# BioJulia/Kmers.jl

Measured on NVIDIA B200. Metric: canonical 31-mers+hash/sec, higher is better.
Workload: dtype u64

## Files before the change

### kmers.jl_b200/csrc/api.cu

```cuda
#include <algorithm>
#include <cstdio>
#include <cstring>
#include <new>
#include <vector>

#include "fourbit.h"
#include "plan.h"

namespace kmc {

int32_t fail_cuda(kmc_ctx *ctx, cudaError_t e, const char *what)
{
    if (ctx) {
        char buf[512];
        snprintf(buf, sizeof buf, "%s: %s (%s)", what, cudaGetErrorName(e), cudaGetErrorString(e));
        ctx->last_error = buf;
    }
    return -static_cast<int32_t>(e);
}

int32_t fail(kmc_ctx *ctx, int32_t code, const char *msg)
{
    if (ctx) ctx->last_error = msg;
    return code;
}

ExtractLaunchFn get_launcher(const Geometry &ge, int mode, bool hash, bool ragged)
{
    switch (ge.n_limbs) {
    case 1: return get_extract_launcher_n1(ge.nx, mode, hash, ragged);
    case 2: return get_extract_launcher_n2(ge.nx, mode, hash, ragged);
    case 3: return get_extract_launcher_n3(ge.nx, mode, hash, ragged);
    case 4: return get_extract_launcher_n4(ge.nx, mode, hash, ragged);
    }
    return nullptr;
}

ExtractLaunchFn get_digest_launcher(const Geometry &ge, int mode, bool hash, bool ragged)
{
    switch (ge.n_limbs) {
    case 1: return get_digest_launcher_n1(ge.nx, mode, hash, ragged);
    case 2: return get_digest_launcher_n2(ge.nx, mode, hash, ragged);
    }
    return nullptr;
}

namespace {

bool aligned32(const void *p) { return (reinterpret_cast<uintptr_t>(p) & 31) == 0; }

__global__ void fill_uniform_offsets_kernel(uint64_t *out, uint64_t n_plus_1, uint64_t step)
{
    uint64_t i = static_cast<uint64_t>(blockIdx.x) * blockDim.x + threadIdx.x;
    if (i < n_plus_1) out[i] = i * step;
}

}

cudaError_t fill_uniform_offsets(uint64_t *out, uint64_t n_plus_1, uint64_t step, cudaStream_t stream)
{
    fill_uniform_offsets_kernel<<<static_cast<unsigned>((n_plus_1 + 255) / 256), 256, 0, stream>>>(out, n_plus_1, step);
    return cudaGetLastError();
}

int32_t check_common(kmc_ctx *ctx, const kmc_seqs *s, int32_t k)
{
    if (!ctx) return KMC_E_BAD_ARG;
    if (!s) return fail(ctx, KMC_E_BAD_ARG, "kmc_seqs is NULL");
    if (k < 1) return fail(ctx, KMC_E_BAD_K, "K must be at least 1");
    if (k > KMC_MAX_K) return fail(ctx, KMC_E_BAD_K, "K exceeds KMC_MAX_K (128)");
    if (s->src_bits != 2 && s->src_bits != 4 && s->src_bits != 8)
        return fail(ctx, KMC_E_BAD_ARG, "src_bits must be 2, 4 (LongSequence words) or 8 (ASCII bytes)");
    if (s->n_seqs > 0 && s->words == nullptr && s->n_words > 0) return fail(ctx, KMC_E_BAD_ARG, "words is NULL");
    return KMC_OK;
}

uint64_t layout_scratch_bytes(const kmc_seqs *s)
{
    if (s->seq_len == nullptr) return 0;
    const uint64_t n = s->n_seqs;
    return 4 * round_up((n + 1) * 8, 256) + round_up(scan_tmp_elems(n) * 8, 256) +
           round_up((tiles_upper_bound(s) + 1) * 8, 256);
}

int32_t plan_layout(kmc_ctx *ctx, const kmc_seqs *s, int k, const Geometry &ge, cudaStream_t stream,
                    const KnownTotals &known, Scratch &scratch, Layout *L)
{
    L->uniform_len = (s->seq_len == nullptr);
    L->uniform_off = (s->seq_word_offset == nullptr);
    const uint64_t G = static_cast<uint64_t>(ge.g);
    if (L->uniform_len) {
        L->wpr = s->uniform_len >= static_cast<uint64_t>(k) ? s->uniform_len - k + 1 : 0;
        L->total = L->wpr * s->n_seqs;
        L->gprm = (L->wpr % G == 0) ? L->wpr / G : (L->wpr + G - 1) / G + 1;
        if (s->n_seqs == 1) L->gprm = (L->wpr + G - 1) / G;
        L->items = L->gprm * s->n_seqs;
        return KMC_OK;
    }
    const uint64_t n = s->n_seqs;
    uint64_t *cnt = static_cast<uint64_t *>(scratch.take((n + 1) * 8));
    uint64_t *win_off = static_cast<uint64_t *>(scratch.take((n + 1) * 8));
    uint64_t *slots = static_cast<uint64_t *>(scratch.take((n + 1) * 8));
    uint64_t *item_off = static_cast<uint64_t *>(scratch.take((n + 1) * 8));
    uint64_t *tmp = static_cast<uint64_t *>(scratch.take(scan_tmp_elems(n) * 8));
    if (!cnt || !win_off || !slots || !item_off || !tmp) return fail(ctx, KMC_E_BAD_ARG, "internal: scratch window too small");
    CU(window_counts(s->seq_len, n, k, cnt, stream));
    CU(inclusive_offsets_u64(cnt, win_off, n, tmp, stream));
    CU(group_slots(win_off, n, ge.g, slots, stream));
    CU(inclusive_offsets_u64(slots, item_off, n, tmp, stream));
    L->win_off = win_off;
    L->item_off = item_off;
    L->wpr = 0;
    L->gprm = 1;
    if (known.valid) {
        L->total = known.windows;
        L->items = known.items;
    } else {
        uint64_t h[2] = {0, 0};
        CU(cudaMemcpyAsync(&h[0], win_off + n, sizeof(uint64_t), cudaMemcpyDeviceToHost, stream));
        CU(cudaMemcpyAsync(&h[1], item_off + n, sizeof(uint64_t), cudaMemcpyDeviceToHost, stream));
        CU(cudaStreamSynchronize(stream));
        L->total = h[0];
        L->items = h[1];
    }
    const uint64_t tiles = (L->items + kTileItems - 1) / kTileItems;
    if (tiles) {
        uint64_t *tile_first = static_cast<uint64_t *>(scratch.take((tiles + 1) * 8));
        if (!tile_first) return fail(ctx, KMC_E_BAD_ARG, "internal: scratch window too small");
        CU(tile_first_reads(item_off, n, kTileItems, tiles, tile_first, stream));
        L->tile_first = tile_first;
    }
    return KMC_OK;
}

ExtractParams base_params(const kmc_seqs *s, int k, const Geometry &ge, const Layout &L, uint64_t unit_bias)
{
    ExtractParams p;
    memset(&p, 0, sizeof p);
    p.w32 = reinterpret_cast<const uint32_t *>(s->words);
    p.nw32 = static_cast<int64_t>(s->n_words) * 2;
    p.unit_bits = 64;
    p.unit_bias = unit_bias;
    p.first = s->first_symbol_offset;
    p.k = k;
    p.s0 = ge.s0;
    p.head_mask = ge.head_mask;
    p.n_seqs = s->n_seqs;
    p.items = L.items;
    p.stride_units = s->uniform_stride_words;
    p.wpr = L.wpr;
    p.gprm = L.gprm;
    p.seq_unit_off = s->seq_word_offset;
    p.win_off = L.win_off;
    p.item_off = L.item_off;
    p.tile_first = L.tile_first;
    return p;
}

int32_t bind_outputs(kmc_ctx *ctx, const kmc_out *out, int mode, uint32_t flags, ExtractParams *p)
{
    const bool hash = (flags & KMC_HASH_FX) != 0;
    const bool aos = (flags & KMC_AOS) != 0;
    const bool want_index = (mode == KMC_UNAMBIG);
    if (!out->a) return fail(ctx, KMC_E_BAD_ARG, "out.a is NULL");
    if (mode == KMC_FWRV && !aos && !out->b) return fail(ctx, KMC_E_BAD_ARG, "out.b is NULL (FWRV, SoA)");
    if (hash && !out->hash) return fail(ctx, KMC_E_BAD_ARG, "out.hash is NULL (KMC_HASH_FX)");
    if (want_index && !aos && !out->index) return fail(ctx, KMC_E_BAD_ARG, "out.index is NULL (UNAMBIG, SoA)");
    p->out_a = out->a;
    p->out_b = out->b;
    p->out_hash = hash ? out->hash : nullptr;
    p->out_index = want_index ? (aos ? reinterpret_cast<int64_t *>(out->a) : out->index) : nullptr;
    p->index_base = out->index_base;
    p->aos = aos ? 1u : 0u;
    p->vec_ok = aligned32(out->a) && (!p->out_b || aligned32(p->out_b)) && (!p->out_hash || aligned32(p->out_hash)) &&
                (!p->out_index || aligned32(p->out_index));
    return KMC_OK;
}

uint64_t extract_scratch_bytes(const kmc_seqs *s, int k, int mode)
{
    if (s->src_bits != 2) return fourbit_scratch_bytes(s, k, mode);
    return layout_scratch_bytes(s) + 256;
}

int32_t extract_device(kmc_ctx *ctx, const kmc_seqs *s, int32_t k, int32_t mode, uint32_t flags, const kmc_out *out,
                       kmc_result *res, cudaStream_t stream, const KnownTotals &known, uint64_t unit_bias, bool sync,
                       Scratch &scratch)
{
    const Geometry ge = geometry(k);
    const bool hash = (flags & KMC_HASH_FX) != 0;
    const int kmode = (mode == KMC_UNAMBIG) ? MODE_FW : mode;

    if (sync) CU(cudaEventRecord(ctx->ev_k0, stream));
    if ((flags & KMC_AOS) && (mode == KMC_FWRV || mode == KMC_UNAMBIG) && ge.n_limbs == 1 && !s->seq_len && !s->seq_word_offset) {
        const Geometry g2 = geometry(k, 2, kAosGroup);
        Layout L2;
        int32_t st2 = plan_layout(ctx, s, k, g2, stream, known, scratch, &L2);
        if (st2) return st2;
        AosLaunchFn afn = get_aos_launcher_n1(g2.nx, mode == KMC_FWRV, hash);
        if (afn && L2.total > 0 && L2.total <= out->capacity) {
            ExtractParams p2 = base_params(s, k, g2, L2, unit_bias);
            st2 = bind_outputs(ctx, out, mode, flags, &p2);
            if (st2) return st2;
            const cudaError_t e = afn(p2, stream);
            if (e == cudaSuccess) {
                res->n_written = L2.total;
                if (out->seq_out_offset) CU(fill_uniform_offsets(out->seq_out_offset, s->n_seqs + 1, L2.wpr, stream));
                if (sync) {
                    CU(cudaEventRecord(ctx->ev_k1, stream));
                    CU(cudaStreamSynchronize(stream));
                    CU(cudaEventElapsedTime(&res->kernel_ms, ctx->ev_k0, ctx->ev_k1));
                }
                return KMC_OK;
            }
            if (e != cudaErrorNotSupported) return fail_cuda(ctx, e, "launch_extract_aos");
            (void)cudaGetLastError();
        }
    }
    Layout L;
    int32_t st = plan_layout(ctx, s, k, ge, stream, known, scratch, &L);
    if (st) return st;
    res->n_written = L.total;
    if (out->seq_out_offset) {
        if (L.uniform_len)
            CU(fill_uniform_offsets(out->seq_out_offset, s->n_seqs + 1, L.wpr, stream));
        else
            CU(cudaMemcpyAsync(out->seq_out_offset, L.win_off, (s->n_seqs + 1) * sizeof(uint64_t), cudaMemcpyDeviceToDevice, stream));
    }
    if (L.total == 0) return KMC_OK;
    if (L.total > out->capacity) return fail(ctx, KMC_E_OUT_TOO_SMALL, "output capacity smaller than the number of k-mers");
    ExtractParams p = base_params(s, k, ge, L, unit_bias);
    st = bind_outputs(ctx, out, mode, flags, &p);
    if (st) return st;

    const bool fused_digest = known.digest && digest_fusable(s, ge.n_limbs, mode, flags);
    if (fused_digest) p.digest = known.digest;
    ExtractLaunchFn fn = fused_digest ? get_digest_launcher(ge, kmode, hash, !L.uniform_len) : get_launcher(ge, kmode, hash, !L.uniform_len);
    if (!fn) return fail(ctx, KMC_E_UNSUPPORTED, "no kernel for this K");
    CU(fn(p, ctx->sm_count, stream));
    if (sync) {
        CU(cudaEventRecord(ctx->ev_k1, stream));
        CU(cudaStreamSynchronize(stream));
        CU(cudaEventElapsedTime(&res->kernel_ms, ctx->ev_k0, ctx->ev_k1));
    }
    return KMC_OK;
}

int32_t ensure_scratch(kmc_ctx *ctx, uint64_t bytes)
{
    if (bytes <= ctx->scratch_bytes) return KMC_OK;
    if (ctx->scratch) {
        CU(cudaStreamSynchronize(ctx->stream));
        for (int i = 0; i < 3; ++i) CU(cudaStreamSynchronize(ctx->pipe_streams[i]));
        CU(cudaFree(ctx->scratch));
        ctx->scratch = nullptr;
        ctx->scratch_bytes = 0;
    }
    uint64_t want = bytes + bytes / 4 + 4096;
    CU(cudaMalloc(&ctx->scratch, want));
    ctx->scratch_bytes = want;
    return KMC_OK;
}

int32_t ensure_host_small(kmc_ctx *ctx)
{
    if (ctx->host_small) return KMC_OK;
    CU(cudaHostAlloc(reinterpret_cast<void **>(&ctx->host_small), 4096, cudaHostAllocDefault));
    memset(ctx->host_small, 0, 4096);
    CU(cudaMalloc(reinterpret_cast<void **>(&ctx->dev_small), 128));
    return KMC_OK;
}

}

using namespace kmc;

extern "C" {

int32_t kmc_version(void) { return KMC_VERSION; }

int32_t kmc_device_count(int32_t *n)
{
    if (!n) return KMC_E_BAD_ARG;
    int c = 0;
    cudaError_t e = cudaGetDeviceCount(&c);
    if (e != cudaSuccess) {
        *n = 0;
        return (e == cudaErrorNoDevice || e == cudaErrorInsufficientDriver) ? KMC_E_NO_DEVICE : -static_cast<int32_t>(e);
    }
    *n = c;
    return KMC_OK;
}

int32_t kmc_ctx_create(int32_t device, kmc_ctx **out)
{
    if (!out) return KMC_E_BAD_ARG;
    *out = nullptr;
    int32_t n = 0;
    int32_t st = kmc_device_count(&n);
    if (st) return st;
    if (n == 0 || device < 0 || device >= n) return KMC_E_NO_DEVICE;
    kmc_ctx *ctx = new (std::nothrow) kmc_ctx();
    if (!ctx) return KMC_E_BAD_ARG;
    ctx->device = device;
    cudaError_t e = cudaSetDevice(device);
    if (e == cudaSuccess) e = cudaDeviceGetAttribute(&ctx->sm_count, cudaDevAttrMultiProcessorCount, device);
    if (e == cudaSuccess) {
        cudaMemPoolProps props;
        memset(&props, 0, sizeof props);
        props.allocType = cudaMemAllocationTypePinned;
        props.handleTypes = cudaMemHandleTypeNone;
        props.location.type = cudaMemLocationTypeDevice;
        props.location.id = device;
        if (cudaMemPoolCreate(&ctx->pool, &props) == cudaSuccess) {
            uint64_t keep = ~0ull;
            cudaMemPoolSetAttribute(ctx->pool, cudaMemPoolAttrReleaseThreshold, &keep);
        } else {
            ctx->pool = nullptr;
        }
        (void)cudaGetLastError();
    }
    if (e == cudaSuccess) e = cudaStreamCreateWithFlags(&ctx->own_stream, cudaStreamNonBlocking);
    for (int i = 0; i < 3 && e == cudaSuccess; ++i) e = cudaStreamCreateWithFlags(&ctx->pipe_streams[i], cudaStreamNonBlocking);
    if (e == cudaSuccess) e = cudaEventCreate(&ctx->ev_begin);
    if (e == cudaSuccess) e = cudaEventCreate(&ctx->ev_end);
    if (e == cudaSuccess) e = cudaEventCreate(&ctx->ev_k0);
    if (e == cudaSuccess) e = cudaEventCreate(&ctx->ev_k1);
    if (e != cudaSuccess) {
        delete ctx;
        return -static_cast<int32_t>(e);
    }
    ctx->stream = ctx->own_stream;
    *out = ctx;
    return KMC_OK;
}

int32_t kmc_ctx_destroy(kmc_ctx *ctx)
{
    if (!ctx) return KMC_OK;
    cudaSetDevice(ctx->device);
    cudaStreamSynchronize(ctx->stream);
    if (ctx->scratch) cudaFree(ctx->scratch);
    if (ctx->host_small) cudaFreeHost(ctx->host_small);
    if (ctx->dev_small) cudaFree(ctx->dev_small);
    for (int i = 0; i < 3; ++i) {
        if (ctx->pipe_buf[i]) cudaFree(ctx->pipe_buf[i]);
        if (ctx->pipe_streams[i]) cudaStreamDestroy(ctx->pipe_streams[i]);
        if (ctx->pipe_events[i]) cudaEventDestroy(ctx->pipe_events[i]);
    }
    if (ctx->ev_begin) cudaEventDestroy(ctx->ev_begin);
    if (ctx->ev_end) cudaEventDestroy(ctx->ev_end);
    if (ctx->ev_k0) cudaEventDestroy(ctx->ev_k0);
    if (ctx->ev_k1) cudaEventDestroy(ctx->ev_k1);
    if (ctx->comm) comm_detach(ctx);
    if (ctx->own_stream) cudaStreamDestroy(ctx->own_stream);
    if (ctx->pool) cudaMemPoolDestroy(ctx->pool);
    delete ctx;
    return KMC_OK;
}

int32_t kmc_ctx_set_stream(kmc_ctx *ctx, void *cuda_stream)
{
    if (!ctx) return KMC_E_BAD_ARG;
    ctx->stream = cuda_stream ? static_cast<cudaStream_t>(cuda_stream) : ctx->own_stream;
    return KMC_OK;
}

int32_t kmc_sync(kmc_ctx *ctx)
{
    if (!ctx) return KMC_E_BAD_ARG;
    CU(cudaSetDevice(ctx->device));
    CU(cudaStreamSynchronize(ctx->stream));
    return KMC_OK;
}

int32_t kmc_trim(kmc_ctx *ctx)
{
    if (!ctx) return KMC_E_BAD_ARG;
    CU(cudaSetDevice(ctx->device));
    CU(cudaStreamSynchronize(ctx->stream));
    for (int i = 0; i < 3; ++i) CU(cudaStreamSynchronize(ctx->pipe_streams[i]));
    if (ctx->pool) CU(cudaMemPoolTrimTo(ctx->pool, 0));
    return KMC_OK;
}

const char *kmc_last_error(kmc_ctx *ctx) { return ctx ? ctx->last_error.c_str() : "kmc_ctx is NULL"; }

const char *kmc_status_string(int32_t status)
{
    switch (status) {
    case KMC_OK: return "ok";
    case KMC_E_BAD_K: return "K must be at least 1 (and at most KMC_MAX_K)";
    case KMC_E_BAD_ARG: return "bad argument";
    case KMC_E_AMBIGUOUS: return "cannot encode an uncertain symbol in a 2-bit alphabet";
    case KMC_E_OUT_TOO_SMALL: return "output buffer too small";
    case KMC_E_NO_DEVICE: return "no CUDA device";
    case KMC_E_UNSUPPORTED: return "unsupported configuration";
    case KMC_E_NCCL: return "NCCL error (or NCCL could not be loaded)";
    }
    if (status < 0) return cudaGetErrorString(static_cast<cudaError_t>(-status));
    return "unknown status";
}

int32_t kmc_device_info(kmc_ctx *ctx, int32_t *sm_count, uint64_t *total_mem, char *name, int32_t name_len)
{
    if (!ctx) return KMC_E_BAD_ARG;
    cudaDeviceProp prop;
    CU(cudaGetDeviceProperties(&prop, ctx->device));
    if (sm_count) *sm_count = prop.multiProcessorCount;
    if (total_mem) *total_mem = prop.totalGlobalMem;
    if (name && name_len > 0) {
        strncpy(name, prop.name, static_cast<size_t>(name_len) - 1);
        name[name_len - 1] = 0;
    }
    return KMC_OK;
}

int32_t kmc_malloc(kmc_ctx *ctx, uint64_t bytes, void **dptr)
{
    if (!ctx || !dptr) return KMC_E_BAD_ARG;
    CU(cudaSetDevice(ctx->device));
    CU(cudaMalloc(dptr, bytes ? bytes : 1));
    return KMC_OK;
}

int32_t kmc_free(kmc_ctx *ctx, void *dptr)
{
    if (!ctx) return KMC_E_BAD_ARG;
    if (!dptr) return KMC_OK;
    CU(cudaSetDevice(ctx->device));
    CU(cudaFree(dptr));
    return KMC_OK;
}

int32_t kmc_memset(kmc_ctx *ctx, void *dptr, int32_t value, uint64_t bytes)
{
    if (!ctx) return KMC_E_BAD_ARG;
    if (bytes == 0) return KMC_OK;
    CU(cudaSetDevice(ctx->device));
    CU(cudaMemsetAsync(dptr, value, bytes, ctx->stream));
    return KMC_OK;
}

int32_t kmc_upload(kmc_ctx *ctx, void *dptr, const void *host, uint64_t bytes)
{
    if (!ctx) return KMC_E_BAD_ARG;
    if (bytes == 0) return KMC_OK;
    CU(cudaSetDevice(ctx->device));
    CU(cudaMemcpyAsync(dptr, host, bytes, cudaMemcpyHostToDevice, ctx->stream));
    return KMC_OK;
}

int32_t kmc_download(kmc_ctx *ctx, void *host, const void *dptr, uint64_t bytes)
{
    if (!ctx) return KMC_E_BAD_ARG;
    CU(cudaSetDevice(ctx->device));
    if (bytes) CU(cudaMemcpyAsync(host, dptr, bytes, cudaMemcpyDeviceToHost, ctx->stream));
    CU(cudaStreamSynchronize(ctx->stream));
    return KMC_OK;
}

int32_t kmc_host_alloc(kmc_ctx *ctx, uint64_t bytes, void **hptr)
{
    if (!ctx || !hptr) return KMC_E_BAD_ARG;
    CU(cudaSetDevice(ctx->device));
    CU(cudaHostAlloc(hptr, bytes ? bytes : 1, cudaHostAllocDefault));
    return KMC_OK;
}

int32_t kmc_host_free(kmc_ctx *ctx, void *hptr)
{
    if (!ctx) return KMC_E_BAD_ARG;
    if (!hptr) return KMC_OK;
    CU(cudaFreeHost(hptr));
    return KMC_OK;
}

int32_t kmc_host_register(kmc_ctx *ctx, void *hptr, uint64_t bytes)
{
    if (!ctx || !hptr) return KMC_E_BAD_ARG;
    CU(cudaSetDevice(ctx->device));
    CU(cudaHostRegister(hptr, bytes, cudaHostRegisterDefault));
    return KMC_OK;
}

int32_t kmc_host_unregister(kmc_ctx *ctx, void *hptr)
{
    if (!ctx || !hptr) return KMC_E_BAD_ARG;
    CU(cudaHostUnregister(hptr));
    return KMC_OK;
}

int32_t kmc_count(kmc_ctx *ctx, const kmc_seqs *seqs, int32_t k, int32_t mode, uint64_t *n_out)
{
    int32_t st = check_common(ctx, seqs, k);
    if (st) return st;
    if (!n_out) return fail(ctx, KMC_E_BAD_ARG, "n_out is NULL");
    if (mode < KMC_FW || mode > KMC_UNAMBIG) return fail(ctx, KMC_E_BAD_ARG, "unknown mode");
    CU(cudaSetDevice(ctx->device));
    if (mode == KMC_UNAMBIG && seqs->src_bits != 2) return count_unambiguous_4bit(ctx, seqs, k, n_out, ctx->stream);
    const Geometry ge = geometry(k);
    st = ensure_scratch(ctx, layout_scratch_bytes(seqs) + 256);
    if (st) return st;
    Scratch scratch{static_cast<char *>(ctx->scratch), ctx->scratch_bytes, 0};
    Layout L;
    st = plan_layout(ctx, seqs, k, ge, ctx->stream, KnownTotals(), scratch, &L);
    if (st) return st;
    *n_out = L.total;
    return KMC_OK;
}

int32_t kmc_extract(kmc_ctx *ctx, const kmc_seqs *seqs, int32_t k, int32_t mode, uint32_t flags, const kmc_out *out,
                    kmc_result *result)
{
    int32_t st = check_common(ctx, seqs, k);
    if (st) return st;
    if (!out || !result) return fail(ctx, KMC_E_BAD_ARG, "kmc_out / kmc_result is NULL");
    if (mode < KMC_FW || mode > KMC_UNAMBIG) return fail(ctx, KMC_E_BAD_ARG, "unknown mode");
    CU(cudaSetDevice(ctx->device));
    result->n_written = 0;
    result->err_seq = result->err_pos = 0;
    result->err_sym = 0;
    result->kernel_ms = 0.f;
    if (flags & KMC_KMER4) {
        st = check_kmer4(ctx, seqs, k, mode);
        if (st) return st;
        st = ensure_scratch(ctx, kmer4_scratch_bytes(seqs));
        if (st) return st;
        Scratch scratch{static_cast<char *>(ctx->scratch), ctx->scratch_bytes, 0};
        return extract_device_kmer4(ctx, seqs, k, mode, flags, out, result, ctx->stream, KnownTotals(), 0,
                                    (flags & KMC_NO_SYNC) == 0, scratch);
    }
    if (seqs->src_bits != 2) return extract_device_4bit(ctx, seqs, k, mode, flags, out, result, ctx->stream);
    st = ensure_scratch(ctx, extract_scratch_bytes(seqs, k, mode));
    if (st) return st;
    Scratch scratch{static_cast<char *>(ctx->scratch), ctx->scratch_bytes, 0};
    return extract_device(ctx, seqs, k, mode, flags, out, result, ctx->stream, KnownTotals(), 0,
                          (flags & KMC_NO_SYNC) == 0, scratch);
}

int32_t kmc_fx_hash(kmc_ctx *ctx, const uint64_t *kmers, uint64_t n, int32_t n_limbs, uint64_t h0, uint64_t *out)
{
    if (!ctx) return KMC_E_BAD_ARG;
    if (n_limbs < 0 || n_limbs > 4) return fail(ctx, KMC_E_BAD_ARG, "n_limbs must be in 0..4");
    if (n && (!out || (n_limbs && !kmers))) return fail(ctx, KMC_E_BAD_ARG, "NULL buffer");
    CU(cudaSetDevice(ctx->device));
    CU(launch_fx_hash(kmers, n, n_limbs, h0, out, ctx->sm_count, ctx->stream));
    return KMC_OK;
}

int32_t kmc_base_hash(kmc_ctx *ctx, const uint64_t *kmers, uint64_t n, int32_t n_limbs, int32_t k, uint64_t h0, uint64_t *out)
{
    if (!ctx) return KMC_E_BAD_ARG;
    if (n_limbs < 0 || n_limbs > 4) return fail(ctx, KMC_E_BAD_ARG, "n_limbs must be in 0..4");
    if (k < 0) return fail(ctx, KMC_E_BAD_K, "K must not be negative");
    if (n && (!out || (n_limbs && !kmers))) return fail(ctx, KMC_E_BAD_ARG, "NULL buffer");
    CU(cudaSetDevice(ctx->device));
    CU(launch_base_hash(kmers, n, n_limbs, h0 ^ static_cast<uint64_t>(k), out, ctx->sm_count, ctx->stream));
    return KMC_OK;
}

namespace {
int32_t bucket_count_impl(kmc_ctx *ctx, const kmc_seqs *seqs, int32_t k, int32_t bucket_bits, uint32_t *table, uint32_t n_parts,
                          void *const *events, kmc_result *result);
}

int32_t kmc_bucket_count(kmc_ctx *ctx, const kmc_seqs *seqs, int32_t k, int32_t bucket_bits, uint32_t *table,
                         kmc_result *result)
{
    return bucket_count_impl(ctx, seqs, k, bucket_bits, table, 0, nullptr, result);
}

int32_t kmc_bucket_count_async(kmc_ctx *ctx, const kmc_seqs *seqs, int32_t k, int32_t bucket_bits, uint32_t *table,
                               uint32_t n_parts, void *const *events, kmc_result *result)
{
    if (!ctx) return KMC_E_BAD_ARG;
    if (!events || n_parts < 1 || n_parts > 32 || (n_parts & (n_parts - 1)))
        return fail(ctx, KMC_E_BAD_ARG, "n_parts must be a power of two <= 32 and events non-NULL");
    for (uint32_t i = 0; i < n_parts; ++i)
        if (!events[i]) return fail(ctx, KMC_E_BAD_ARG, "NULL event");
    return bucket_count_impl(ctx, seqs, k, bucket_bits, table, n_parts, events, result);
}

namespace {
int32_t bucket_count_impl(kmc_ctx *ctx, const kmc_seqs *seqs, int32_t k, int32_t bucket_bits, uint32_t *table, uint32_t n_parts,
                          void *const *events, kmc_result *result)
{
    int32_t st = check_common(ctx, seqs, k);
    if (st) return st;
    if (!table || !result) return fail(ctx, KMC_E_BAD_ARG, "table / result is NULL");
    if (bucket_bits < 1 || bucket_bits > 32) return fail(ctx, KMC_E_BAD_ARG, "bucket_bits must be in 1..32");
    if (seqs->src_bits != 2) return fail(ctx, KMC_E_UNSUPPORTED, "bucket count needs a 2-bit source");
    CU(cudaSetDevice(ctx->device));
    result->n_written = 0;
    result->err_seq = result->err_pos = 0;
    result->err_sym = 0;
    result->kernel_ms = 0.f;
    const Geometry ge = geometry(k);
    cudaStream_t stream = ctx->stream;
    CU(cudaEventRecord(ctx->ev_k0, stream));
    st = ensure_scratch(ctx, layout_scratch_bytes(seqs) + 256);
    if (st) return st;
    Scratch scratch{static_cast<char *>(ctx->scratch), ctx->scratch_bytes, 0};
    Layout L;
    st = plan_layout(ctx, seqs, k, ge, stream, KnownTotals(), scratch, &L);
    if (st) return st;
    result->n_written = L.total;
    auto record_all = [&]() -> int32_t {
        for (uint32_t i = 0; i < n_parts; ++i) CU(cudaEventRecord(static_cast<cudaEvent_t>(events[i]), stream));
        return KMC_OK;
    };
    if (L.total == 0) return record_all();
    ExtractParams p = base_params(seqs, k, ge, L, 0);
    p.bucket_shift = static_cast<uint32_t>(64 - bucket_bits);
    const uint64_t table_bytes = 4ull << bucket_bits;
    const bool want_binned = table_bytes > (96ull << 20) && bucket_bits <= 32;

    auto count_direct = [&](ExtractParams q, cudaStream_t s) -> int32_t {
        int32_t rc = ensure_host_small(ctx);
        if (rc) return rc;
        if (table_bytes <= (96ull << 20)) CU(warm_table(table, 1ull << bucket_bits, ctx->sm_count, warm_sink(ctx), s));
        q.bucket_table = table;
        ExtractLaunchFn fn = get_launcher(ge, MODE_BUCKETS, true, !L.uniform_len);
        if (!fn) return fail(ctx, KMC_E_UNSUPPORTED, "no kernel for this K");
        CU(fn(q, ctx->sm_count, s));
        return KMC_OK;
    };
    auto count_exact = [&](ExtractParams q, uint64_t windows, cudaStream_t s, uint32_t np, void *const *ev) -> int32_t {
        AsyncBuf ids_buf, tmp_buf, matrix_buf, offs_buf, scan_buf;
        const uint64_t n_ids = (q.items + 1) * static_cast<uint64_t>(ge.g);
        const uint64_t cells = (static_cast<uint64_t>(1) << binned_count_bin_bits(bucket_bits)) * binned_count_blocks(n_ids);
        cudaError_t e = ids_buf.alloc(ctx, round_up(n_ids * 4, 256), s);
        if (e == cudaSuccess) e = tmp_buf.alloc(ctx, round_up(n_ids * 4, 256), s);
        if (e == cudaSuccess) e = matrix_buf.alloc(ctx, (cells + 1) * 8, s);
        if (e == cudaSuccess) e = offs_buf.alloc(ctx, (cells + 2) * 8, s);
        if (e == cudaSuccess) e = scan_buf.alloc(ctx, (scan_tmp_elems(cells) + 1) * 8, s);
        if (e != cudaSuccess) {
            (void)cudaGetLastError();
            int32_t rc = count_direct(q, s);
            if (rc) return rc;
            for (uint32_t i = 0; i < np; ++i) CU(cudaEventRecord(static_cast<cudaEvent_t>(ev[i]), s));
            return KMC_OK;
        }
        q.out_a = ids_buf.as<uint64_t>();
        q.vec_ok = 1;
        ExtractLaunchFn fn = get_launcher(ge, MODE_BUCKET_IDS, true, !L.uniform_len);
        if (!fn) return fail(ctx, KMC_E_UNSUPPORTED, "no kernel for this K");
        CU(fn(q, ctx->sm_count, s));
        CU(binned_count(ids_buf.as<uint32_t>(), windows, bucket_bits, table, tmp_buf.as<uint32_t>(), matrix_buf.as<uint64_t>(),
                        offs_buf.as<uint64_t>(), scan_buf.as<uint64_t>(), ctx->sm_count, s, np, ev));
        return KMC_OK;
    };

    bool done = false;
    ExtractParams pa = p;
    if (want_binned) set_iteration_strides(pa, ge.g);
    if (want_binned && ge.n_limbs == 1 && L.uniform_len && binned_count_bin_bits(bucket_bits) == 6 && fused_bin_enabled() && pa.aligned &&
        pa.al_tail == 0 && pa.items < 0xffffffffull - kTileItems) {
        AsyncBuf bins_buf, state_buf;
        const uint64_t cap = fused_bin_capacity(L.total);
        cudaError_t e = bins_buf.alloc(ctx, fused_bin_buffer_ids(L.total) * 4, stream);
        if (e == cudaSuccess) e = state_buf.alloc(ctx, fused_bin_state_bytes(), stream);
        if (e != cudaSuccess) {
            (void)cudaGetLastError();
        } else {
            st = ensure_host_small(ctx);
            if (st) return st;
            CU(fused_bin_ids(pa, ge.nx, bucket_bits, bins_buf.as<uint32_t>(), cap, state_buf.as<unsigned long long>(), stream));
            CU(fused_bin_apply(bins_buf.as<uint32_t>(), cap, state_buf.as<unsigned long long>(), bucket_bits, table, warm_sink(ctx),
                               ctx->sm_count, stream, n_parts, events));
            done = true;
        }
    }
    if (!done && want_binned) {
        st = count_exact(p, L.total, stream, n_parts, events);
        if (st) return st;
        done = true;
    }
    if (!done) {
        st = count_direct(p, stream);
        if (st) return st;
        st = record_all();
        if (st) return st;
    }
    if (n_parts) return KMC_OK;
    CU(cudaEventRecord(ctx->ev_k1, stream));
    CU(cudaStreamSynchronize(stream));
    CU(cudaEventElapsedTime(&result->kernel_ms, ctx->ev_k0, ctx->ev_k1));
    return KMC_OK;
}
}

int32_t kmc_digest(kmc_ctx *ctx, const uint64_t *dptr, uint64_t n, uint64_t *out)
{
    if (!ctx) return KMC_E_BAD_ARG;
    if (!out || (n && !dptr)) return fail(ctx, KMC_E_BAD_ARG, "NULL buffer");
    CU(cudaSetDevice(ctx->device));
    int32_t st = ensure_scratch(ctx, 256);
    if (st) return st;
    uint64_t *acc = static_cast<uint64_t *>(ctx->scratch);
    CU(launch_digest(dptr, n, acc, ctx->sm_count, ctx->stream));
    CU(cudaMemcpyAsync(out, acc, 16, cudaMemcpyDeviceToHost, ctx->stream));
    CU(cudaStreamSynchronize(ctx->stream));
    return KMC_OK;
}

int32_t kmc_timer_begin(kmc_ctx *ctx)
{
    if (!ctx) return KMC_E_BAD_ARG;
    CU(cudaSetDevice(ctx->device));
    CU(cudaEventRecord(ctx->ev_begin, ctx->stream));
    return KMC_OK;
}

int32_t kmc_timer_end(kmc_ctx *ctx, float *ms)
{
    if (!ctx || !ms) return KMC_E_BAD_ARG;
    CU(cudaSetDevice(ctx->device));
    CU(cudaEventRecord(ctx->ev_end, ctx->stream));
    CU(cudaEventSynchronize(ctx->ev_end));
    CU(cudaEventElapsedTime(ms, ctx->ev_begin, ctx->ev_end));
    return KMC_OK;
}

int32_t kmc_store_probe(kmc_ctx *ctx, void *dptr, uint64_t bytes)
{
    if (!ctx || !dptr) return KMC_E_BAD_ARG;
    CU(cudaSetDevice(ctx->device));
    CU(launch_store_probe(dptr, bytes, ctx->sm_count, ctx->stream));
    return KMC_OK;
}

}
```

### kmers.jl_b200/csrc/buckets.cu

```cuda
#include <cstdlib>
#include <type_traits>

#include "binning.cuh"
#include "plan.h"

namespace kmc {

namespace {

__global__ void __launch_bounds__(256) warm_slice_kernel(const uint32_t *__restrict__ slice, uint64_t n_counters,
                                                         uint32_t *__restrict__ sink)
{
    const uint4 *p = reinterpret_cast<const uint4 *>(slice);
    const uint64_t n4 = n_counters / 4;
    uint32_t acc = 0;
    for (uint64_t i = static_cast<uint64_t>(blockIdx.x) * blockDim.x + threadIdx.x; i < n4;
         i += static_cast<uint64_t>(gridDim.x) * blockDim.x) {
        uint4 v;
        asm volatile("ld.global.L1::no_allocate.L2::cache_hint.v4.u32 {%0,%1,%2,%3}, [%4], %5;"
                     : "=r"(v.x), "=r"(v.y), "=r"(v.z), "=r"(v.w)
                     : "l"(p + i), "l"(0x14F0000000000000ull));
        acc |= v.x & v.y & v.z & v.w;
    }
    if (acc == 0xffffffffu) *sink = acc;
}

__global__ void __launch_bounds__(256) bin_apply_kernel(const uint32_t *__restrict__ binned, const uint64_t *__restrict__ offs,
                                                        uint64_t n_blocks, int bin, int bin_end, uint32_t *__restrict__ table)
{
    const uint64_t begin = __ldg(offs + static_cast<uint64_t>(bin) * n_blocks);
    const uint64_t end = __ldg(offs + static_cast<uint64_t>(bin_end) * n_blocks);
    const uint64_t a4 = (begin + 3) & ~3ull;
    const uint64_t tid = static_cast<uint64_t>(blockIdx.x) * blockDim.x + threadIdx.x;
    const uint64_t threads = static_cast<uint64_t>(gridDim.x) * blockDim.x;
    if (tid < a4 - begin && begin + tid < end) atomicAdd(table + binned[begin + tid], 1u);
    for (uint64_t i = a4 + tid * 4; i < end; i += threads * 4) {
        if (i + 4 <= end) {
            const uint4 v = __ldg(reinterpret_cast<const uint4 *>(binned + i));
            atomicAdd(table + v.x, 1u);
            atomicAdd(table + v.y, 1u);
            atomicAdd(table + v.z, 1u);
            atomicAdd(table + v.w, 1u);
        } else {
            for (uint64_t j = i; j < end; ++j) atomicAdd(table + binned[j], 1u);
        }
    }
}


constexpr int kStateBinEnd = binning::kTpBins;
constexpr int kStateSpill = 2 * binning::kTpBins;
constexpr int kStateWords = 2 * binning::kTpBins + 2;

struct FusedBins {
    uint32_t *binned;
    uint64_t cap;
    unsigned long long *state;
    int bin_shift;
};

template <int NX>
__global__ void __launch_bounds__(binning::kBlock, 3) bucket_bin_kernel(const ExtractParams p, const FusedBins f)
{
    using S = binning::Shape<uint32_t>;
    constexpr int G = 8, PT = S::kPerThread;
    static_assert(PT == 2 * G && S::kChunk == kTileItems * G, "a thread bins the ids of two work items per iteration");
    extern __shared__ __align__(16) unsigned char smem_raw[];
    binning::Scatter64Smem<uint32_t> &sm = *reinterpret_cast<binning::Scatter64Smem<uint32_t> *>(smem_raw);
    const uint32_t n_items = static_cast<uint32_t>(p.items);
    const uint32_t tile_base = blockIdx.x * static_cast<uint32_t>(kTileItems);
    if (p.pf_tiles) burst_prefetch<false, G, 2>(p, n_items);
    const AlignedItems<G, 2> items(p);
    const uint32_t tile_end = n_items - tile_base > static_cast<uint32_t>(kTileItems) ? tile_base + kTileItems : n_items;
    const bool inside = items.template loads_inside<NX>(p, tile_end - 1u);
    const binning::IdBin bin_of{f.bin_shift};
    constexpr int kItemsPerIter = 2 * binning::kBlock;
    auto reserve = [&](int b, uint32_t count) -> uint64_t {
        if (count == 0) return 0;
        const uint64_t at = atomicAdd(f.state + b, static_cast<unsigned long long>(count));
        if (at + count > f.cap) {
            atomicMin(f.state + kStateBinEnd + b, static_cast<unsigned long long>(at));
            return binning::kTpBins * f.cap + atomicAdd(f.state + kStateSpill, static_cast<unsigned long long>(count));
        }
        return static_cast<uint64_t>(b) * f.cap + at;
    };
    auto ids_of = [&](uint32_t item, uint32_t *key) {
        uint32_t x[NX];
        load_block_at<NX>(p, items.bit_of(item), inside, x);
        uint64_t fw[G][1], rv[G][1];
        block_kmers<1, NX, G, true, true, 2>(x, p.s0, p.head_mask, fw, rv);
#pragma unroll
        for (int j = 0; j < G; ++j) {
            const uint64_t c[1] = {fw[j][0] < rv[j][0] ? fw[j][0] : rv[j][0]};
            key[j] = static_cast<uint32_t>(fx_hash<1>(c, 0) >> p.bucket_shift);
        }
    };
#pragma unroll 1
    for (uint32_t it_base = tile_base; it_base < tile_end; it_base += kItemsPerIter) {
        uint32_t key[PT];
        if (tile_end - it_base >= static_cast<uint32_t>(kItemsPerIter)) {
            ids_of(it_base + threadIdx.x, key);
            ids_of(it_base + binning::kBlock + threadIdx.x, key + G);
            binning::scatter64_iter<uint32_t, true>(sm, key, 0xffffu, bin_of, reserve, f.binned);
        } else {
            uint32_t ok_mask = 0;
#pragma unroll
            for (int j = 0; j < PT; ++j) key[j] = 0;
            if (it_base + threadIdx.x < tile_end) {
                ids_of(it_base + threadIdx.x, key);
                ok_mask = 0xffu;
            }
            if (it_base + binning::kBlock + threadIdx.x < tile_end) {
                ids_of(it_base + binning::kBlock + threadIdx.x, key + G);
                ok_mask |= 0xff00u;
            }
            binning::scatter64_iter<uint32_t, false>(sm, key, ok_mask, bin_of, reserve, f.binned);
        }
    }
}

__device__ __forceinline__ uint4 ld_ids(const uint32_t *p)
{
    uint4 v;
    asm volatile("ld.global.nc.L1::no_allocate.L2::cache_hint.v4.u32 {%0,%1,%2,%3}, [%4], %5;"
                 : "=r"(v.x), "=r"(v.y), "=r"(v.z), "=r"(v.w)
                 : "l"(p), "l"(0x12F0000000000000ull));
    return v;
}
__device__ __forceinline__ void inc_counter(uint32_t *p)
{
    asm volatile("red.global.add.L2::cache_hint.u32 [%0], 1, %1;" ::"l"(p), "l"(0x14F0000000000000ull) : "memory");
}

__global__ void __launch_bounds__(256) bin_apply_fused_kernel(const uint32_t *__restrict__ binned, uint64_t cap,
                                                              const unsigned long long *__restrict__ state, int bin, int bin_end,
                                                              uint32_t *__restrict__ table)
{
    const uint64_t tid = static_cast<uint64_t>(blockIdx.x) * blockDim.x + threadIdx.x;
    const uint64_t step = static_cast<uint64_t>(gridDim.x) * blockDim.x * 4;
    for (int b = bin; b < bin_end; ++b) {
        const uint32_t *ids = binned + static_cast<uint64_t>(b) * cap;
        const uint64_t reserved = state[b], full_at = state[kStateBinEnd + b];
        const uint64_t n = reserved < full_at ? reserved : full_at, n4 = n & ~3ull;
        uint64_t i = tid * 4;
        uint4 v = make_uint4(0, 0, 0, 0);
        if (i < n4) v = ld_ids(ids + i);
        while (i < n4) {
            const uint64_t nxt = i + step;
            uint4 w = make_uint4(0, 0, 0, 0);
            if (nxt < n4) w = ld_ids(ids + nxt);
            inc_counter(table + v.x);
            inc_counter(table + v.y);
            inc_counter(table + v.z);
            inc_counter(table + v.w);
            v = w;
            i = nxt;
        }
        if (tid < n - n4) inc_counter(table + ids[n4 + tid]);
    }
}

__global__ void __launch_bounds__(256) spill_apply_kernel(const uint32_t *__restrict__ spill, const unsigned long long *__restrict__ state,
                                                          uint32_t *__restrict__ table)
{
    const uint64_t n = state[kStateSpill];
    for (uint64_t i = static_cast<uint64_t>(blockIdx.x) * blockDim.x + threadIdx.x; i < n; i += static_cast<uint64_t>(gridDim.x) * blockDim.x)
        atomicAdd(table + spill[i], 1u);
}

}

cudaError_t binned_count(const uint32_t *ids, uint64_t n, int bucket_bits, uint32_t *table, uint32_t *binned, uint64_t *matrix,
                         uint64_t *offs, uint64_t *scan_tmp, int sm_count, cudaStream_t stream, uint32_t n_parts, void *const *events)
{
    if (!events) n_parts = 0;
    if (n == 0) {
        for (uint32_t i = 0; i < n_parts; ++i) {
            cudaError_t e = cudaEventRecord(static_cast<cudaEvent_t>(events[i]), stream);
            if (e != cudaSuccess) return e;
        }
        return cudaSuccess;
    }
    const int p = binned_count_bin_bits(bucket_bits);
    if (bucket_bits < p) return cudaErrorInvalidValue;
    const int n_bins = 1 << p, shift = bucket_bits - p;
    const uint64_t n_blocks = binned_count_blocks(n);
    cudaError_t e = binning::partition<uint32_t>(ids, n, p, binning::IdBin{shift}, binned, matrix, offs, scan_tmp, stream);
    if (e != cudaSuccess) return e;
    const uint64_t slice = 1ull << shift;
    const int group = apply_group(2);
    uint32_t parts_done = 0;
    for (int b = 0; b < n_bins; b += group) {
        const int b_end = b + group < n_bins ? b + group : n_bins;
        warm_slice_kernel<<<static_cast<unsigned>(sm_count * 8), 256, 0, stream>>>(table + static_cast<uint64_t>(b) * slice,
                                                                                  slice * (b_end - b), reinterpret_cast<uint32_t *>(scan_tmp));
        bin_apply_kernel<<<static_cast<unsigned>(sm_count * 16), 256, 0, stream>>>(binned, offs, n_blocks, b, b_end, table);
        while (parts_done < n_parts && static_cast<uint64_t>(parts_done + 1) * n_bins <= static_cast<uint64_t>(b_end) * n_parts) {
            e = cudaEventRecord(static_cast<cudaEvent_t>(events[parts_done++]), stream);
            if (e != cudaSuccess) return e;
        }
    }
    return cudaGetLastError();
}

uint64_t fused_bin_capacity(uint64_t n_ids)
{
    const uint64_t cap = n_ids / binning::kTpBins + n_ids / (8 * binning::kTpBins) + 8192;
    return (cap + 3) & ~3ull;
}
uint64_t fused_bin_buffer_ids(uint64_t n_ids) { return binning::kTpBins * fused_bin_capacity(n_ids) + n_ids + 4096; }
uint64_t fused_bin_state_bytes() { return kStateWords * sizeof(unsigned long long); }

cudaError_t fused_bin_ids(ExtractParams p, int nx, int bucket_bits, uint32_t *binned, uint64_t cap, unsigned long long *state,
                          cudaStream_t stream)
{
    const int pbits = binned_count_bin_bits(bucket_bits);
    if (pbits != 6 || bucket_bits < pbits) return cudaErrorInvalidValue;
    const uint64_t tiles = (p.items + kTileItems - 1) / kTileItems;
    if (tiles == 0 || tiles > 0x7fffffffull || p.items >= 0xffffffffull - kTileItems) return cudaErrorInvalidConfiguration;
    set_iteration_strides(p, 8);
    if (!p.aligned || p.al_tail) return cudaErrorInvalidValue;
    p.al_magic = aligned_magic(p.gprm);
    p.pf_tiles = 0;
    if (prefetch_enabled()) {
        const uint64_t per_tile = static_cast<uint64_t>(p.nw32) * 4 / tiles + 1, t = kPfChunkBytes / per_tile;
        p.pf_tiles = static_cast<uint32_t>(t < 2 * kPfLead ? 2 * kPfLead : (t > (1u << 20) ? (1u << 20) : t));
    }
    cudaError_t e = cudaMemsetAsync(state, 0, kStateWords * sizeof(unsigned long long), stream);
    if (e == cudaSuccess) e = cudaMemsetAsync(state + kStateBinEnd, 0xff, binning::kTpBins * sizeof(unsigned long long), stream);
    if (e != cudaSuccess) return e;
    const FusedBins f{binned, cap, state, bucket_bits - pbits};
    constexpr int smem = static_cast<int>(sizeof(binning::Scatter64Smem<uint32_t>));
    auto launch = [&](auto tag) -> cudaError_t {
        constexpr int NX = decltype(tag)::value;
        cudaError_t e2 = cudaFuncSetAttribute(bucket_bin_kernel<NX>, cudaFuncAttributeMaxDynamicSharedMemorySize, smem);
        if (e2 != cudaSuccess) return e2;
        bucket_bin_kernel<NX><<<static_cast<unsigned>(tiles), binning::kBlock, smem, stream>>>(p, f);
        return cudaGetLastError();
    };
    switch (nx) {
    case 1: return launch(std::integral_constant<int, 1>());
    case 2: return launch(std::integral_constant<int, 2>());
    case 3: return launch(std::integral_constant<int, 3>());
    }
    return cudaErrorInvalidValue;
}

cudaError_t fused_bin_apply(const uint32_t *binned, uint64_t cap, const unsigned long long *state, int bucket_bits, uint32_t *table,
                            uint32_t *sink, int sm_count, cudaStream_t stream, uint32_t n_parts, void *const *events)
{
    if (!events) n_parts = 0;
    const int pbits = binned_count_bin_bits(bucket_bits);
    const int n_bins = 1 << pbits, shift = bucket_bits - pbits;
    const uint64_t slice = 1ull << shift;
    const int group = apply_group(2);
    spill_apply_kernel<<<static_cast<unsigned>(sm_count * 8), 256, 0, stream>>>(binned + static_cast<uint64_t>(n_bins) * cap, state, table);
    uint32_t parts_done = 0;
    for (int b = 0; b < n_bins; b += group) {
        const int b_end = b + group < n_bins ? b + group : n_bins;
        warm_slice_kernel<<<static_cast<unsigned>(sm_count * 8), 256, 0, stream>>>(table + static_cast<uint64_t>(b) * slice,
                                                                                  slice * (b_end - b), sink);
        bin_apply_fused_kernel<<<static_cast<unsigned>(sm_count * 16), 256, 0, stream>>>(binned, cap, state, b, b_end, table);
        while (parts_done < n_parts && static_cast<uint64_t>(parts_done + 1) * n_bins <= static_cast<uint64_t>(b_end) * n_parts) {
            cudaError_t e = cudaEventRecord(static_cast<cudaEvent_t>(events[parts_done++]), stream);
            if (e != cudaSuccess) return e;
        }
    }
    return cudaGetLastError();
}

bool fused_bin_enabled()
{
    static const bool on = [] {
        const char *e = getenv("KMC_FUSED_BIN");
        return !(e && e[0] == '0');
    }();
    return on;
}

int apply_group(int dflt)
{
    static const int env = [] {
        const char *e = getenv("KMC_APPLY_GROUP");
        const int v = e ? atoi(e) : 0;
        return v < 0 ? 0 : (v > 64 ? 64 : v);
    }();
    return env ? env : dflt;
}

cudaError_t warm_table(const uint32_t *table, uint64_t n_counters, int sm_count, uint32_t *sink, cudaStream_t stream)
{
    warm_slice_kernel<<<static_cast<unsigned>(sm_count * 8), 256, 0, stream>>>(table, n_counters, sink);
    return cudaGetLastError();
}

int binned_count_bin_bits(int bucket_bits)
{
    int p = bucket_bits - 22;
    if (p < binning::kMinBits) p = binning::kMinBits;
    if (p > binning::kMaxBits) p = binning::kMaxBits;
    return p;
}

uint64_t binned_count_blocks(uint64_t n) { return binning::blocks_for<uint32_t>(n); }

}
```

### kmers.jl_b200/csrc/kmc_internal.h

```cpp
#pragma once
#include <cuda_runtime.h>
#include <cstdint>
#include <string>

#include "../../include/kmerscuda.h"

struct kmc_comm;

struct kmc_ctx {
    int device = 0;
    int sm_count = 0;
    cudaStream_t own_stream = nullptr;
    cudaStream_t stream = nullptr;
    cudaStream_t pipe_streams[3] = {nullptr, nullptr, nullptr};
    cudaEvent_t pipe_events[3] = {nullptr, nullptr, nullptr};
    cudaEvent_t ev_begin = nullptr, ev_end = nullptr;
    cudaEvent_t ev_k0 = nullptr, ev_k1 = nullptr;
    void *scratch = nullptr;
    uint64_t scratch_bytes = 0;
    void *pipe_buf[3] = {nullptr, nullptr, nullptr};
    uint64_t pipe_bytes[3] = {0, 0, 0};
    uint64_t *host_small = nullptr;
    uint64_t *dev_small = nullptr;
    cudaMemPool_t pool = nullptr;
    kmc_comm *comm = nullptr;
    std::string last_error;
};

namespace kmc {

struct AsyncBuf {
    void *p = nullptr;
    cudaStream_t s = nullptr;
    cudaError_t alloc(kmc_ctx *ctx, uint64_t bytes, cudaStream_t stream)
    {
        s = stream;
        return ctx->pool ? cudaMallocFromPoolAsync(&p, bytes ? bytes : 1, ctx->pool, stream)
                         : cudaMallocAsync(&p, bytes ? bytes : 1, stream);
    }
    template <typename T> T *as() const { return static_cast<T *>(p); }
    AsyncBuf() = default;
    AsyncBuf(const AsyncBuf &) = delete;
    AsyncBuf &operator=(const AsyncBuf &) = delete;
    ~AsyncBuf()
    {
        if (p) cudaFreeAsync(p, s);
    }
};

inline uint32_t *warm_sink(kmc_ctx *ctx) { return reinterpret_cast<uint32_t *>(ctx->dev_small) + 24; }

void comm_detach(kmc_ctx *ctx);

int32_t ensure_scratch(kmc_ctx *ctx, uint64_t bytes);
int32_t ensure_host_small(kmc_ctx *ctx);

uint64_t scan_tmp_elems(uint64_t n);
cudaError_t inclusive_offsets_u64(const uint64_t *in, uint64_t *out, uint64_t n, uint64_t *tmp, cudaStream_t stream);
cudaError_t window_counts(const uint64_t *seq_len, uint64_t n, int k, uint64_t *cnt, cudaStream_t stream);
cudaError_t group_slots(const uint64_t *win_off, uint64_t n, int g, uint64_t *slots, cudaStream_t stream);

cudaError_t tile_first_reads(const uint64_t *item_off, uint64_t n_seqs, uint64_t tile_items, uint64_t n_tiles,
                             uint64_t *tile_first, cudaStream_t stream);

int binned_count_bin_bits(int bucket_bits);
int apply_group(int dflt);
uint64_t binned_count_blocks(uint64_t n);
cudaError_t warm_table(const uint32_t *table, uint64_t n_counters, int sm_count, uint32_t *sink, cudaStream_t stream);
cudaError_t binned_count(const uint32_t *ids, uint64_t n, int bucket_bits, uint32_t *table, uint32_t *binned, uint64_t *matrix,
                         uint64_t *offs, uint64_t *scan_tmp, int sm_count, cudaStream_t stream, uint32_t n_parts = 0,
                         void *const *events = nullptr);

struct ExtractParams;
bool fused_bin_enabled();
uint64_t fused_bin_capacity(uint64_t n_ids);
uint64_t fused_bin_buffer_ids(uint64_t n_ids);
uint64_t fused_bin_state_bytes();
cudaError_t fused_bin_ids(ExtractParams p, int nx, int bucket_bits, uint32_t *binned, uint64_t cap, unsigned long long *state,
                          cudaStream_t stream);
cudaError_t fused_bin_apply(const uint32_t *binned, uint64_t cap, const unsigned long long *state, int bucket_bits, uint32_t *table,
                            uint32_t *sink, int sm_count, cudaStream_t stream, uint32_t n_parts, void *const *events);

cudaError_t launch_fx_hash(const uint64_t *kmers, uint64_t n, int n_limbs, uint64_t h0, uint64_t *out, int sm_count,
                           cudaStream_t stream);
cudaError_t launch_digest(const uint64_t *p, uint64_t n, uint64_t *acc, int sm_count, cudaStream_t stream, bool zero = true);
cudaError_t launch_base_hash(const uint64_t *kmers, uint64_t n, int n_limbs, uint64_t h, uint64_t *out, int sm_count,
                             cudaStream_t stream);
cudaError_t launch_store_probe(void *dptr, uint64_t bytes, int sm_count, cudaStream_t stream);

}
```

Baseline: 453.8 billion.

## Add second-level sub-binning and shared-memory slice counting for fused bucket apply

New measurement: 453.0 billion, median of 6. No clear change (-0.2%).

```diff
diff --git a/kmers.jl_b200/csrc/api.cu b/kmers.jl_b200/csrc/api.cu
--- a/kmers.jl_b200/csrc/api.cu
+++ b/kmers.jl_b200/csrc/api.cu
@@ -657,10 +657,11 @@
     if (want_binned) set_iteration_strides(pa, ge.g);
     if (want_binned && ge.n_limbs == 1 && L.uniform_len && binned_count_bin_bits(bucket_bits) == 6 && fused_bin_enabled() && pa.aligned &&
         pa.al_tail == 0 && pa.items < 0xffffffffull - kTileItems) {
-        AsyncBuf bins_buf, state_buf;
+        AsyncBuf bins_buf, state_buf, sub_buf;
         const uint64_t cap = fused_bin_capacity(L.total);
         cudaError_t e = bins_buf.alloc(ctx, fused_bin_buffer_ids(L.total) * 4, stream);
         if (e == cudaSuccess) e = state_buf.alloc(ctx, fused_bin_state_bytes(), stream);
+        if (e == cudaSuccess && smem_count_enabled()) e = sub_buf.alloc(ctx, fused_sub_buffer_bytes(cap), stream);
         if (e != cudaSuccess) {
             (void)cudaGetLastError();
         } else {
@@ -668,7 +669,7 @@
             if (st) return st;
             CU(fused_bin_ids(pa, ge.nx, bucket_bits, bins_buf.as<uint32_t>(), cap, state_buf.as<unsigned long long>(), stream));
             CU(fused_bin_apply(bins_buf.as<uint32_t>(), cap, state_buf.as<unsigned long long>(), bucket_bits, table, warm_sink(ctx),
-                               ctx->sm_count, stream, n_parts, events));
+                               ctx->sm_count, stream, n_parts, events, sub_buf.p));
             done = true;
         }
     }
diff --git a/kmers.jl_b200/csrc/buckets.cu b/kmers.jl_b200/csrc/buckets.cu
--- a/kmers.jl_b200/csrc/buckets.cu
+++ b/kmers.jl_b200/csrc/buckets.cu
@@ -160,12 +160,192 @@
     }
 }
 
-__global__ void __launch_bounds__(256) spill_apply_kernel(const uint32_t *__restrict__ spill, const unsigned long long *__restrict__ state,
+__global__ void __launch_bounds__(256) spill_apply_kernel(const uint32_t *__restrict__ spill, const unsigned long long *__restrict__ n_spill,
                                                           uint32_t *__restrict__ table)
 {
-    const uint64_t n = state[kStateSpill];
+    const uint64_t n = *n_spill;
     for (uint64_t i = static_cast<uint64_t>(blockIdx.x) * blockDim.x + threadIdx.x; i < n; i += static_cast<uint64_t>(gridDim.x) * blockDim.x)
         atomicAdd(table + spill[i], 1u);
+}
+
+constexpr int kSubBits = 6, kSubBins = 1 << kSubBits;
+constexpr int kSubAll = binning::kTpBins * kSubBins;
+constexpr int kSub2End = kSubAll;
+constexpr int kSub2Spill = 2 * kSubAll;
+constexpr int kSub2Ticket = kSub2Spill + binning::kTpBins;
+constexpr int kSub2Words = kSub2Ticket + binning::kTpBins;
+constexpr uint64_t kSub2StateBytes = (kSub2Words * sizeof(unsigned long long) + 255) & ~255ull;
+
+constexpr int kSubGroup = 8;
+
+__host__ __device__ __forceinline__ uint64_t sub_bin_capacity(uint64_t n)
+{
+    return (n / kSubBins + n / (8 * kSubBins) + 1024 + 3) & ~3ull;
+}
+
+struct SubBin {
+    int shift;
+    __device__ __forceinline__ uint32_t operator()(uint32_t id) const { return (id >> shift) & (kSubBins - 1); }
+};
+
+struct SubBins {
+    uint32_t *ids;
+    uint64_t region;
+    uint64_t spill_at;
+    unsigned long long *state;
+};
+
+__device__ __forceinline__ uint64_t bin_ids(const unsigned long long *state, int b)
+{
+    const uint64_t reserved = state[b], full_at = state[kStateBinEnd + b];
+    return reserved < full_at ? reserved : full_at;
+}
+
+__global__ void __launch_bounds__(binning::kBlock, 3) subbin_kernel(const uint32_t *__restrict__ binned, uint64_t cap,
+                                                                   const unsigned long long *__restrict__ state, int bin, int bin_end,
+                                                                   int sub_shift, const SubBins s)
+{
+    using S = binning::Shape<uint32_t>;
+    constexpr int PT = S::kPerThread;
+    static_assert(PT == 16 && S::kPerIter == 4 * 4 * binning::kBlock, "a thread loads four 16-byte vectors per iteration");
+    extern __shared__ __align__(16) unsigned char smem_raw[];
+    binning::Scatter64Smem<uint32_t> &sm = *reinterpret_cast<binning::Scatter64Smem<uint32_t> *>(smem_raw);
+    const SubBin sub_of{sub_shift};
+    unsigned long long *spill = s.state + kSub2Spill + bin;
+    for (int b = bin; b < bin_end; ++b) {
+        const uint64_t n = bin_ids(state, b), cap2 = sub_bin_capacity(n);
+        const uint32_t *in = binned + static_cast<uint64_t>(b) * cap;
+        const uint64_t region = static_cast<uint64_t>(b - bin) * s.region;
+        unsigned long long *cursor = s.state + b * kSubBins, *full = s.state + kSub2End + b * kSubBins;
+        auto reserve = [&](int q, uint32_t count) -> uint64_t {
+            if (count == 0) return 0;
+            const uint64_t at = atomicAdd(cursor + q, static_cast<unsigned long long>(count));
+            if (at + count > cap2) {
+                atomicMin(full + q, static_cast<unsigned long long>(at));
+                return s.spill_at + atomicAdd(spill, static_cast<unsigned long long>(count));
+            }
+            return region + static_cast<uint64_t>(q) * cap2 + at;
+        };
+        const uint64_t step = static_cast<uint64_t>(gridDim.x) * S::kPerIter;
+        for (uint64_t it = static_cast<uint64_t>(blockIdx.x) * S::kPerIter; it < n; it += step) {
+            uint32_t key[PT];
+            if (it + step + S::kPerIter <= n) {
+#pragma unroll
+                for (int r = 0; r < 4; ++r)
+                    asm volatile("prefetch.global.L2 [%0];" ::"l"(in + it + step + (r * binning::kBlock + threadIdx.x) * 4));
+            }
+            if (it + S::kPerIter <= n) {
+#pragma unroll
+                for (int r = 0; r < 4; ++r) {
+                    const uint4 v = ld_ids(in + it + (r * binning::kBlock + threadIdx.x) * 4);
+                    key[4 * r + 0] = v.x;
+                    key[4 * r + 1] = v.y;
+                    key[4 * r + 2] = v.z;
+                    key[4 * r + 3] = v.w;
+                }
+                binning::scatter64_iter<uint32_t, true>(sm, key, 0xffffu, sub_of, reserve, s.ids);
+            } else {
+                uint32_t ok_mask = 0;
+#pragma unroll
+                for (int r = 0; r < 4; ++r) {
+                    const uint64_t e = it + (r * binning::kBlock + threadIdx.x) * 4;
+#pragma unroll
+                    for (int q = 0; q < 4; ++q) {
+                        const bool ok = e + q < n;
+                        key[4 * r + q] = ok ? in[e + q] : 0u;
+                        ok_mask |= (ok ? 1u : 0u) << (4 * r + q);
+                    }
+                }
+                binning::scatter64_iter<uint32_t, false>(sm, key, ok_mask, sub_of, reserve, s.ids);
+            }
+        }
+    }
+}
+
+constexpr int kCountThreads = 1024, kRoundVecs = 4, kRound = kRoundVecs * 4 * kCountThreads;
+static_assert(kRound + 3 <= 0x8000, "a round adds less than 0x8000 to a half");
+
+__device__ __forceinline__ bool count_id(uint32_t *w, uint32_t c)
+{
+    const uint32_t sh = (c & 1u) << 4;
+    const uint32_t old = atomicAdd(w + (c >> 1), 1u << sh);
+    return ((old >> sh) & 0xffffu) >= 0x7fffu;
+}
+
+__global__ void __launch_bounds__(kCountThreads, 1) slice_count_kernel(const SubBins s, const unsigned long long *__restrict__ state,
+                                                                       int bin, int bin_end, int slice_bits, uint32_t *__restrict__ table)
+{
+    extern __shared__ __align__(16) uint32_t w[];
+    __shared__ uint32_t s_ticket;
+    const uint32_t n_words = 1u << (slice_bits - 1), mask = (1u << slice_bits) - 1u;
+    const uint32_t n_sub = static_cast<uint32_t>(bin_end - bin) * kSubBins;
+    for (uint32_t i = threadIdx.x; i < n_words; i += kCountThreads) w[i] = 0;
+    for (;;) {
+        if (threadIdx.x == 0) s_ticket = static_cast<uint32_t>(atomicAdd(s.state + kSub2Ticket + bin, 1ull));
+        __syncthreads();
+        const uint32_t t = s_ticket;
+        if (t >= n_sub) break;
+        const int b = bin + static_cast<int>(t / kSubBins), q = static_cast<int>(t % kSubBins);
+        const uint64_t reserved = s.state[b * kSubBins + q], full_at = s.state[kSub2End + b * kSubBins + q];
+        const uint32_t n = static_cast<uint32_t>(reserved < full_at ? reserved : full_at), n4 = n & ~3u;
+        const uint32_t *ids = s.ids + static_cast<uint64_t>(b - bin) * s.region + static_cast<uint64_t>(q) * sub_bin_capacity(bin_ids(state, b));
+        uint32_t *slice = table + (static_cast<uint64_t>(b * kSubBins + q) << slice_bits);
+        bool hot = false;
+        if (threadIdx.x < n - n4) hot = count_id(w, ids[n4 + threadIdx.x] & mask);
+        uint4 cur[kRoundVecs];
+#pragma unroll
+        for (int j = 0; j < kRoundVecs; ++j) {
+            const uint32_t i = (j * kCountThreads + threadIdx.x) * 4;
+            if (i < n4) cur[j] = ld_ids(ids + i);
+        }
+        for (uint32_t r = 0; r < n4; r += kRound) {
+            uint4 nxt[kRoundVecs];
+#pragma unroll
+            for (int j = 0; j < kRoundVecs; ++j) {
+                const uint32_t i = r + kRound + (j * kCountThreads + threadIdx.x) * 4;
+                if (i < n4) nxt[j] = ld_ids(ids + i);
+            }
+#pragma unroll
+            for (int j = 0; j < kRoundVecs; ++j) {
+                if (r + (j * kCountThreads + threadIdx.x) * 4 < n4) {
+                    hot |= count_id(w, cur[j].x & mask);
+                    hot |= count_id(w, cur[j].y & mask);
+                    hot |= count_id(w, cur[j].z & mask);
+                    hot |= count_id(w, cur[j].w & mask);
+                }
+                cur[j] = nxt[j];
+            }
+            if (__syncthreads_or(hot)) {
+                for (uint32_t i = threadIdx.x; i < n_words; i += kCountThreads) {
+                    uint32_t x = w[i];
+                    if (x & 0x8000u) {
+                        atomicAdd(slice + 2 * i, 0x8000u);
+                        x -= 0x8000u;
+                    }
+                    if (x & 0x80000000u) {
+                        atomicAdd(slice + 2 * i + 1, 0x8000u);
+                        x -= 0x80000000u;
+                    }
+                    w[i] = x;
+                }
+                __syncthreads();
+            }
+            hot = false;
+        }
+        __syncthreads();
+        for (uint32_t i = threadIdx.x; i < n_words / 2; i += kCountThreads) {
+            const uint2 a = reinterpret_cast<const uint2 *>(w)[i];
+            reinterpret_cast<uint2 *>(w)[i] = make_uint2(0, 0);
+            uint4 *p = reinterpret_cast<uint4 *>(slice) + i;
+            uint4 v = __ldcg(p);
+            v.x += a.x & 0xffffu;
+            v.y += a.x >> 16;
+            v.z += a.y & 0xffffu;
+            v.w += a.y >> 16;
+            __stcg(p, v);
+        }
+        __syncthreads();
+    }
 }
 
 }
@@ -246,21 +426,52 @@
     return cudaErrorInvalidValue;
 }
 
+uint64_t fused_sub_buffer_bytes(uint64_t cap)
+{
+    const uint64_t group = static_cast<uint64_t>(apply_group(kSubGroup));
+    return kSub2StateBytes + group * (kSubBins * sub_bin_capacity(cap) + cap) * sizeof(uint32_t);
+}
+
 cudaError_t fused_bin_apply(const uint32_t *binned, uint64_t cap, const unsigned long long *state, int bucket_bits, uint32_t *table,
-                            uint32_t *sink, int sm_count, cudaStream_t stream, uint32_t n_parts, void *const *events)
+                            uint32_t *sink, int sm_count, cudaStream_t stream, uint32_t n_parts, void *const *events, void *sub)
 {
     if (!events) n_parts = 0;
     const int pbits = binned_count_bin_bits(bucket_bits);
     const int n_bins = 1 << pbits, shift = bucket_bits - pbits;
     const uint64_t slice = 1ull << shift;
-    const int group = apply_group(2);
-    spill_apply_kernel<<<static_cast<unsigned>(sm_count * 8), 256, 0, stream>>>(binned + static_cast<uint64_t>(n_bins) * cap, state, table);
+    const int group = apply_group(sub ? kSubGroup : 2);
+    SubBins s{};
+    constexpr int sub_smem = static_cast<int>(sizeof(binning::Scatter64Smem<uint32_t>));
+    const int slice_bits = shift - kSubBits, count_smem = 2 << slice_bits;
+    if (sub) {
+        if (pbits != 6 || slice_bits < 2 || count_smem > (128 << 10)) return cudaErrorInvalidValue;
+        s.state = static_cast<unsigned long long *>(sub);
+        s.ids = reinterpret_cast<uint32_t *>(static_cast<char *>(sub) + kSub2StateBytes);
+        s.region = kSubBins * sub_bin_capacity(cap);
+        s.spill_at = static_cast<uint64_t>(group) * s.region;
+        cudaError_t e = cudaMemsetAsync(s.state, 0, kSub2Words * sizeof(unsigned long long), stream);
+        if (e == cudaSuccess) e = cudaMemsetAsync(s.state + kSub2End, 0xff, kSubAll * sizeof(unsigned long long), stream);
+        if (e == cudaSuccess) e = cudaFuncSetAttribute(subbin_kernel, cudaFuncAttributeMaxDynamicSharedMemorySize, sub_smem);
+        if (e == cudaSuccess) e = cudaFuncSetAttribute(slice_count_kernel, cudaFuncAttributeMaxDynamicSharedMemorySize, count_smem);
+        if (e != cudaSuccess) return e;
+    }
+    spill_apply_kernel<<<static_cast<unsigned>(sm_count * 8), 256, 0, stream>>>(binned + static_cast<uint64_t>(n_bins) * cap,
+                                                                               state + kStateSpill, table);
     uint32_t parts_done = 0;
     for (int b = 0; b < n_bins; b += group) {
         const int b_end = b + group < n_bins ? b + group : n_bins;
-        warm_slice_kernel<<<static_cast<unsigned>(sm_count * 8), 256, 0, stream>>>(table + static_cast<uint64_t>(b) * slice,
-                                                                                  slice * (b_end - b), sink);
-        bin_apply_fused_kernel<<<static_cast<unsigned>(sm_count * 16), 256, 0, stream>>>(binned, cap, state, b, b_end, table);
+        if (sub) {
+            subbin_kernel<<<static_cast<unsigned>(sm_count * 3), binning::kBlock, sub_smem, stream>>>(binned, cap, state, b, b_end,
+                                                                                                     slice_bits, s);
+            spill_apply_kernel<<<static_cast<unsigned>(sm_count * 8), 256, 0, stream>>>(s.ids + s.spill_at, s.state + kSub2Spill + b,
+                                                                                       table);
+            slice_count_kernel<<<static_cast<unsigned>(sm_count), kCountThreads, count_smem, stream>>>(s, state, b, b_end, slice_bits,
+                                                                                                       table);
+        } else {
+            warm_slice_kernel<<<static_cast<unsigned>(sm_count * 8), 256, 0, stream>>>(table + static_cast<uint64_t>(b) * slice,
+                                                                                      slice * (b_end - b), sink);
+            bin_apply_fused_kernel<<<static_cast<unsigned>(sm_count * 16), 256, 0, stream>>>(binned, cap, state, b, b_end, table);
+        }
         while (parts_done < n_parts && static_cast<uint64_t>(parts_done + 1) * n_bins <= static_cast<uint64_t>(b_end) * n_parts) {
             cudaError_t e = cudaEventRecord(static_cast<cudaEvent_t>(events[parts_done++]), stream);
             if (e != cudaSuccess) return e;
@@ -276,6 +487,12 @@
         return !(e && e[0] == '0');
     }();
     return on;
+}
+
+bool smem_count_enabled()
+{
+    const char *e = getenv("KMC_SMEM_COUNT");
+    return !(e && e[0] == '0');
 }
 
 int apply_group(int dflt)
diff --git a/kmers.jl_b200/csrc/kmc_internal.h b/kmers.jl_b200/csrc/kmc_internal.h
--- a/kmers.jl_b200/csrc/kmc_internal.h
+++ b/kmers.jl_b200/csrc/kmc_internal.h
@@ -78,8 +78,10 @@
 uint64_t fused_bin_state_bytes();
 cudaError_t fused_bin_ids(ExtractParams p, int nx, int bucket_bits, uint32_t *binned, uint64_t cap, unsigned long long *state,
                           cudaStream_t stream);
+bool smem_count_enabled();
+uint64_t fused_sub_buffer_bytes(uint64_t cap);
 cudaError_t fused_bin_apply(const uint32_t *binned, uint64_t cap, const unsigned long long *state, int bucket_bits, uint32_t *table,
-                            uint32_t *sink, int sm_count, cudaStream_t stream, uint32_t n_parts, void *const *events);
+                            uint32_t *sink, int sm_count, cudaStream_t stream, uint32_t n_parts, void *const *events, void *sub);
 
 cudaError_t launch_fx_hash(const uint64_t *kmers, uint64_t n, int n_limbs, uint64_t h0, uint64_t *out, int sm_count,
                            cudaStream_t stream);
```
